# sebhaan/geobo

Hardware: AMD Instinct MI355X
Metric: voxels/sec posterior (mean+var) for 64^3 x 2-prop joint inversion; fp64 roofline % (higher is better)
Workload: dtype f64

## Files before the change

geobo_amd/_lib.py:

```python
import ctypes as C
import os

LIB_PATH = os.environ.get("GEOBO_HIP_LIB") or os.path.join(os.path.dirname(os.path.abspath(__file__)), "lib", "libgeobo_hip.so")

_dp = C.c_void_p
_i64 = C.c_int64
_f64 = C.c_double
_int = C.c_int
_sz = C.c_size_t

SIGNATURES = {
    "geobo_version": (_int, []),
    "geobo_pad_m": (_i64, [_i64]),
    "geobo_pad_n": (_i64, [_i64]),
    "geobo_k_block": (_int, [_int, _dp, _dp, _dp, _i64, _dp, _dp, _dp, _i64, _f64, _f64, _f64, _f64, _dp, _i64, _dp]),
    "geobo_k_block_f32": (_int, [_int, _dp, _dp, _dp, _i64, _dp, _dp, _dp, _i64, _f64, _f64, _f64, _f64, _dp, _i64, _dp]),
    "geobo_k_block_grid": (_int, [_int, _int, _int, _dp, _dp, _i64, _i64, _i64, _i64, _int, _dp, _i64, _dp]),
    "geobo_lattice_wbuild": (_int, [_i64, _int, _int, _int, _dp, _dp, _dp, _dp]),
    "geobo_lattice_wplanes": (_int, [_i64, _int, _int, _int, _dp, _dp, _dp, _dp]),
    "geobo_xz2d_fold_inv_strided": (_int, [_int, _i64, _int, _dp, _i64, _i64, _dp, _dp, _dp, _i64, _i64, _i64, _dp]),
    "geobo_xz2d_fold_inv_mul": (_int, [_int, _i64, _int, _dp, _i64, _dp, _i64, _dp, _dp, _dp, _i64, _i64, _i64, _dp]),
    "geobo_xz2d_fold_conv_fwd": (_int, [_int, _i64, _int, _dp, _i64, _dp, _i64, _dp, _i64, _dp, _dp, _dp, _i64, _i64, _dp]),
    "geobo_sumsq_accum": (_int, [_i64, _i64, _dp, _i64, _dp, _i64, _int, _dp, _i64, _dp]),
    "geobo_lamdot_z": (_int, [_i64, _int, _int, _int, _dp, _dp, _dp, _dp]),
    "geobo_centro_fill": (_int, [_dp, _i64, _i64, _i64, _dp]),
    "geobo_transpose": (_int, [_i64, _i64, _dp, _i64, _dp, _i64, _dp]),
    "geobo_mirror_rows": (_int, [_dp, _i64, _i64, _i64, _i64, _int, _dp]),
    "geobo_mirror_planes": (_int, [_dp, _i64, _dp, _i64, _i64, _i64, _i64, _int, _int, _dp]),
    "geobo_mirror_dev_ws_bytes": (_sz, []),
    "geobo_mirror_dev": (_int, [_dp, _i64, _dp, _i64, _i64, _int, _int, _dp, _dp, _sz, _dp]),
    "geobo_colgemv_ws_bytes": (_sz, [_i64, _i64]),
    "geobo_colgemv": (_int, [_i64, _i64, _dp, _i64, _dp, _dp, _dp, _sz, _dp]),
    "geobo_rowgemv": (_int, [_i64, _i64, _dp, _i64, _dp, _dp, _dp]),
    "geobo_convert": (_int, [_int, _dp, _i64, _dp, _i64, _i64, _i64, _dp]),
    "geobo_round_f32": (_int, [_dp, _i64, _dp]),
    "geobo_k_eval": (_int, [_int, _dp, _i64, _f64, _f64, _f64, _f64, _dp, _dp]),
    "geobo_a_sens": (_int, [_int, C.POINTER(_f64), _dp, _i64, _int, _int, _int, _dp, _dp, _dp, _f64, _f64, _dp, _i64, _dp]),
    "geobo_a_sens_slab": (_int, [_int, C.POINTER(_f64), _dp, _i64, _int, _int, _int, _dp, _dp, _dp, _f64, _f64, _int, _int, _dp, _i64, _i64, _dp]),
    "geobo_potential": (_int, [_int, C.POINTER(_f64), _dp, _dp, _dp, _i64, _dp, _dp]),
    "geobo_ak_fused": (_int, [_int, _dp, _i64, _i64, _i64, _dp, _dp, _dp, _i64, _i64, _f64, _f64, _f64, _f64, _dp, _i64, _dp]),
    "geobo_ak_points": (_int, [_int, _dp, _i64, _i64, _i64, _dp, _dp, _dp, _dp, _dp, _dp, _i64, _f64, _f64, _f64, _f64, _dp, _i64, _dp]),
    "geobo_cov_table": (_int, [_int, _int, _int, _int, _f64, _f64, _f64, _f64, _f64, _f64, _f64, _dp, _dp]),
    "geobo_ak_fused_grid": (_int, [_dp, _i64, _i64, _i64, _int, _int, _int, _dp, _i64, _i64, _dp, _i64, _dp]),
# ... 119 lines not shown
```

geobo_amd/csrc/reduce.hip:

```cpp
#include <hip/hip_runtime.h>
#include <stdint.h>
#include "geobo_hip.h"

namespace {

typedef double v2d __attribute__((ext_vector_type(2)));

__global__ void __launch_bounds__(256) sumsq_accum_kernel(int64_t rows, int64_t n2, const double* __restrict__ a, int64_t lda,
                                                          const double* __restrict__ b, int64_t ldb, int slots, double* __restrict__ ss,
                                                          int64_t ld_ss) {
  const int64_t c2 = (int64_t)blockIdx.x * 256 + threadIdx.x;
  if (c2 >= n2) return;
  const int slot = blockIdx.y;
  v2d acc = *reinterpret_cast<const v2d*>(ss + slot * ld_ss + 2 * c2);
  if (b) {
    for (int64_t r = slot; r < rows; r += slots) {
      const v2d x = *reinterpret_cast<const v2d*>(a + r * lda + 2 * c2) + *reinterpret_cast<const v2d*>(b + r * ldb + 2 * c2);
      acc.x = __builtin_fma(x.x, x.x, acc.x);
      acc.y = __builtin_fma(x.y, x.y, acc.y);
    }
  } else {
    for (int64_t r = slot; r < rows; r += slots) {
      const v2d x = *reinterpret_cast<const v2d*>(a + r * lda + 2 * c2);
      acc.x = __builtin_fma(x.x, x.x, acc.x);
// ... 146 lines not shown

__global__ void __launch_bounds__(256) transpose_kernel(int64_t rows, int64_t cols, const double* __restrict__ src, int64_t lds,
                                                        double* __restrict__ dst, int64_t ldd) {
  __shared__ double t[64][65];
  const int tx = threadIdx.x & 63, ty = threadIdx.x >> 6;
  const int64_t r0 = (int64_t)blockIdx.y * 64, c0 = (int64_t)blockIdx.x * 64;
#pragma unroll 4
  for (int i = ty; i < 64; i += 4)
    if (r0 + i < rows && c0 + tx < cols) t[i][tx] = src[(r0 + i) * lds + c0 + tx];
  __syncthreads();
#pragma unroll 4
  for (int i = ty; i < 64; i += 4)
    if (c0 + i < cols && r0 + tx < rows) dst[(c0 + i) * ldd + r0 + tx] = t[tx][i];
}

}

extern "C" int geobo_transpose(int64_t rows, int64_t cols, const double* src, int64_t lds, double* dst, int64_t ldd, void* stream) {
  if (!src || !dst || rows < 0 || cols < 0 || lds < cols || ldd < rows || (rows + 63) / 64 > 65535) return GEOBO_E_ARG;
  if (rows == 0 || cols == 0) return GEOBO_OK;
  hipLaunchKernelGGL(transpose_kernel, dim3((unsigned)((cols + 63) / 64), (unsigned)((rows + 63) / 64)), dim3(256), 0, (hipStream_t)stream,
                     rows, cols, src, lds, dst, ldd);
  return hipGetLastError() == hipSuccess ? GEOBO_OK : GEOBO_E_LAUNCH;
}

extern "C" int geobo_centro_fill(double* B, int64_t ld, int64_t n, int64_t r0, void* stream) {
  if (!B || ((uintptr_t)B & 15) || n < 0 || r0 < 0 || r0 > n || 2 * r0 < n || ld < n) return GEOBO_E_ARG;
  if (ld & 1) return GEOBO_E_ALIGN;
  if (r0 == n) return GEOBO_OK;
  const int64_t gy = n - r0 < 65535 ? n - r0 : 65535;
// ... 76 lines not shown
```

geobo_amd/csrc/toeplitz.hip:

```cpp
#include <hip/hip_runtime.h>
#include <atomic>
#include <stdint.h>
#include "geobo_hip.h"
#include "lds_optin.h"

namespace {

struct ToeplitzArgs {
  const double* in;
  const double* tab[2];
  double* out[2];
  int64_t C, S, R;
  int nprop, y0, y1;
};

using rsrc_t = __amdgpu_buffer_rsrc_t;
using u32x2 = decltype(__builtin_amdgcn_raw_buffer_load_b64(*static_cast<rsrc_t*>(nullptr), 0, 0, 0));
__device__ __forceinline__ rsrc_t make_rsrc(const double* base, int bytes) {
  return __builtin_amdgcn_make_buffer_rsrc(const_cast<double*>(base), 0, bytes, 0x00020000);
}
__device__ __forceinline__ double ld_lane(rsrc_t rs, unsigned lane8, int soff) {
  return __builtin_bit_cast(double, __builtin_amdgcn_raw_buffer_load_b64(rs, lane8, soff, 0));
}
__device__ __forceinline__ void st_lane(rsrc_t rs, unsigned lane8, int soff, double v) {
// ... 590 lines not shown
  if (C <= 0 || C % 64 || (plane & 1) || (int64_t)ny * plane * 8 >= (1ll << 31)) return GEOBO_E_ALIGN;
  if (ny <= 64) {
    for (int j = 0; j < nprop; j += 2) {
      const int n = nprop - j >= 2 ? 2 : 1;
      const int rc = geobo_toeplitz_y(ny, C, plane, R, n, in, tabs[j], n == 2 ? tabs[j + 1] : nullptr, outs[j], n == 2 ? outs[j + 1] : nullptr,
                                      y0, y1, stream);
      if (rc) return rc;
    }
    return GEOBO_OK;
  }
  ToeplitzWinArgs g;
  g.in = in; g.C = C; g.S = plane; g.R = R; g.nprop = nprop; g.y0 = y0; g.y1 = y1;
  for (int j = 0; j < 3; ++j) { g.tab[j] = tabs[j < nprop ? j : 0]; g.out[j] = outs[j < nprop ? j : 0]; }
  return launch_win_by_ny<false>(ny, g, (hipStream_t)stream);
}
```

geobo_amd/engine.py:

```python
import math
import os
import time

import numpy as np
import torch

from . import geometry, hip
from .plan import COLUMN_FORM_MAX_BYTES, cross_options, cross_rows_route, engine_options, feed_options, gram_gx_route, plan_route
from .columnform import ColumnExchangeMixin
from .rowform import RowFormMixin
from .operators import StreamedOperator
from .transposed import TransposedPosteriorMixin
from .information import SetStatisticsMixin
from .crossval import CrossValidationMixin
from .blocksupport import BlockSupportMixin
from .pointpred import PointPredictionMixin
from .resources import ResourceMixin
from .geobodies import GeobodyMixin
from .intercepts import InterceptMixin
from .append import AppendRowsMixin
from .reweight import ReweightMixin
from .step import Prior, Step
from .sharding import (EmulatedGroup, allreduce_sum_, assemble_columns, backend_of, exchange_blocks, exchange_blocks_finish,
                       exchange_blocks_start, gather_rows, gather_slices, shard_columns)
# ... 119 lines not shown
        self._A = {}
        self._ws = {}
        self._host = {}
        self._auto_denied = set()
        self._pending_exchange = None
        self.use_grid = self.nz >= 16 and self.nz % 2 == 0
        if method not in ("auto", "dense", "spectral"):
            raise ValueError("method must be 'auto', 'dense' or 'spectral'")
        self.method = method
        env = os.environ
        self.route = plan_route(self.nx, self.ny, self.nz, world=world, rank=rank, assembly=assembly, operators=operators, method=method,
                                env=env)
        self.options = engine_options(env)
        self.feed = feed_options(env)
        self.cross = cross_options(env)
        self.use_spectral = self.route.spectral
        if method == "spectral" and not self.use_spectral:
            raise ValueError("spectral method needs grid extents % 16 == 0 and column shards on y-slab boundaries")
        if self.route.operators == "streamed":
            self.streamed = True
        if self.route.note and self.N >= 32768:
            import warnings
            warnings.warn("geobo_amd route %s: %s" % (self.route.describe(), self.route.note), RuntimeWarning, stacklevel=3)
        self._spectral = None
        self._lattice_plan = None
        self._gram, self._lam, self._edgeV = None, {}, {}
        self._lamW, self._edgeVt = {}, {}
        self.aka_mirror_on = self.options.aka_mirror
        self.aka_mirror, self._mirror, self._mirror_meas = {}, {}, None
        self.z_spectrum_on = self.options.z_spectrum
# ... 386 lines not shown
        if self.exchange:
            return self._assemble_AK_spectral_exchange(step, AK)
        kept = ((0, 0), (0, 1), (1, 1))
        run = ((0, 0), (1, 0), (1, 1)) if step.cross_rows == "magn" else kept
        for s_, A in ((0, A_g), (1, A_m)):
            gen_of, out_of = {}, {}
            for jj, j in enumerate(props):
                gen_of[j] = sp.eigenvalues(step.prior.table(self, s_, j))
                step.gens[(s_, j)] = gen_of[j]
                out_of[j] = AK[s_ * self.Ms_pad:s_ * self.Ms_pad + self.Ms, jj * nc:(jj + 1) * nc]
            blocks = [j for j in props if not step.sym or (s_, j) in run]
            lams, outs = [gen_of[j] for j in blocks], [out_of[j] for j in blocks]
            pooled = (isinstance(A, StreamedOperator) and A.lattice is not None and A.lattice.jy is not None and not self.f32
                      and sp.pool_applies())
            Mrun = step.mirror if (s_ == 1 and step.mirror) else self.Ms
            fl = sp.flops(Mrun, len(lams), y1 - y0, fwd_planes=sp.pool_planes(Mrun) if pooled else None)
            fv = sp.flops_valu(Mrun, len(lams), y1 - y0)
            feed = self._gram_feed(step, s_, blocks) if (y0, y1) == (0, self.ny) else None
            if feed is not None:
                fl += self._gram.flops_gx(Mrun * len(lams))

            def product_rows(gx, A=A, lams=lams, outs=outs, Mrun=Mrun, pooled=pooled):
                if not self.f32 and not isinstance(A, StreamedOperator):
                    return sp.product(A, Mrun, lams, [o[:Mrun] for o in outs], y0, y1, gx=gx)
                Rb = sp.R
                abuf = self._op_rows_buffer() if isinstance(A, StreamedOperator) else None
                scr = [self._workspace2d("ak_rows64_%d" % jj, Rb, nc) for jj in range(len(lams))] if self.f32 else None
                pool = sp.plane_pool(A.lattice, Mrun, A.lattice.jy, A.lattice.jx) if pooled else None
                for r0 in range(0, Mrun, Rb):
                    R = min(Rb, Mrun - r0)
                    if pool is not None:
                        src = pool.rows(r0)
                    elif abuf is not None and A.lattice is not None:
                        src = A.lattice.rows(r0)
                    else:
                        src = A.rows_into(abuf, r0, R) if abuf is not None else A[r0:r0 + R]
                    dst = [b[:R] for b in scr] if scr is not None else [o[r0:r0 + R] for o in outs]
                    sp.product(src, R, lams, dst, y0, y1, gx=gx and gx.at(r0))
                    if scr is not None:
                        for jj in range(len(lams)):
                            hip.convert(dst[jj], outs[jj][r0:r0 + R])
            self._timed("spectral_product", fl, lambda: product_rows(feed), valu=fv)
            whole = feed is None or feed.store_all
            late = [j for j in props if (not step.sym or (s_, j) in kept) and not (whole and j in blocks)]
            if late:
                step.ak_fill.append(lambda fill=product_rows, lams=[gen_of[j] for j in late], outs=[out_of[j] for j in late]:
                                    fill(None, lams=lams, outs=outs))

    def _gram_feed(self, step, s_, blocks):
        gram, sp = self._gram, self._spectral_product()
        funcs = ("grav", "magn")
        if not (gram_gx_route(self.feed, self.route.family, step.sym, self.f32, self.world, self.exchange, self.nx, self.ny, self.nz, sp.forms)
                and gram is not None and gram.gx_applies() and sp.gx_applies() and all(j in (0, 1) and self._lam.get(funcs[j]) is not None for j in blocks)):
            return None
        S = [self._workspace("gram_S_%d%d" % (s_, j), (self.Ms * gram.Py * gram.Px,)) for j in blocks]
        for j, Sj in zip(blocks, S):
            step.gram_S[(s_, j)] = Sj
        return _GramFeed(gram, [self._lam[funcs[j]][1] for j in blocks], S, store_all=False)

    def _edge_spectrum(self, func, k, ycols):
        key = (func, k)
        hit = self._edgeV.get(key)
        if hit is None or hit[0] != ycols.data_ptr():
            hit = self._edgeV[key] = (ycols.data_ptr(), self._gram.edge_eigen(ycols))
        return hit[1]

    MIRROR_BOUND = 2.0 ** -48

    def _mirror_static(self, plan):
        return bool(self.aka_mirror_on and plan is not None and plan["rowmajor"] and self.route.family == "single" and self.world == 1
# ... 190 lines not shown
                  props=(0, 1, 2), calclogl=True, want_mean_var=True, keep_K=False, potrf_schedule=None):
        props = tuple(props)
        assert 0 in props and 1 in props, "gravity and magnetic blocks are needed for AkA"
        sel = np.asarray(sel, dtype=np.int64)
        sel_t = torch.as_tensor(sel, device=self.device) if sel.size else None
        t = self._tick("start")
        scales = self._step_row_scale(sel)
        y = self._pad_y(y_g, y_m, y_d, hip.pad_m(2 * self.Ms_pad + len(sel)), None if scales is None else scales[1])
        if self.rows_static and not self._rows_denied and not self._rows_ok(A_g, A_m) and all(f in self._op_args for f in ("grav", "magn")):
            A_g, A_m = (self.operator(f, *self._op_args[f][:1], B=self._op_args[f][1], axes=self._op_args[f][2]) for f in ("grav", "magn"))
        step = self._step = self._new_step(Prior(kernelfunc, lengths, weight_matrix(crossweights), gp_amp), props, sel_t, gp_sigma,
                                           keep_signal=bool(keep_K), row_scale=scales, sym=not self.rows_static and self._sym_ok(A_g, A_m))
        M_pad = step.M_pad
        step.mirror = self._mirror_rows(step, A_m)
        step.cross_rows = "magn" if cross_rows_route(self.cross, step.sym, step.mirror, self.nx, self.ny, self.nz) else "grav"
        for f, rec in self.aka_mirror.items():
            rec["taken"] = bool(f == "magn" and step.mirror)
        AK = self._assemble_AK(step, A_g, A_m)
        self.step_route = "rows" if step.rowpath else ("single" if step.sym else "columns")
        t = self._tick("ak_fused", t)
        AkA = self._assemble_AkA(step, AK, A_g, A_m)
        if self.aka_hook is not None:
            self.aka_hook(AkA)
        t = self._tick("aka", t)
        if self._potrf_ctx is None:
            self._potrf_ctx = hip.PotrfContext()
        Linv, info = self._timed("potrf_inv", 2.0 * M_pad ** 3 / 3.0, lambda: hip.potrf_inv(
            AkA, self._workspace("Linv", (M_pad, M_pad)), self._workspace("potrf_ws", (hip.potrf_ws_doubles(M_pad),)),
            ctx=self._potrf_ctx, schedule=potrf_schedule or self.options.potrf), alg=(2 * self.Ms + len(sel)) ** 3 * 2.0 / 3.0)
        L = AkA
        if scales is not None and scales[1].size:
            Linv.diagonal()[torch.as_tensor(scales[1], device=self.device)] = 0.0
# ... 228 lines not shown
```

geobo_amd/hip.py:

```python
import ctypes as C

import numpy as np
import torch

from . import _lib

F64 = torch.float64

KERNEL_IDS = {"d2": 0, "exp": 1, "exp_x": 2, "matern32": 3, "matern32_x": 4, "sparse": 5, "sparse_x": 6,
              "exp_dl": 7, "exp_x_dl1": 8, "exp_x_dl2": 9, "matern32_dl": 10, "matern32_x_dl1": 11, "matern32_x_dl2": 12,
              "sparse_dl": 13, "sparse_x_dl1": 14, "sparse_x_dl2": 15}
FUNC_IDS = {"grav": 0, "magn": 1}
from .plan import (PAD_M, PAD_N, SPECTRAL_AXIS_N, SPECTRAL_Y3T_NY, SPECTRAL_Y_NY, TOEPLITZ_ADD_NY, TOEPLITZ_NY, TOEPLITZ_Y2T_NY,
                   XZ2D_FOLD_N, XZ2D_SHAPES, YMUL_SHAPES)


def kernel_id(name, cross, deriv=None):
    if name not in ("exp", "matern32", "sparse"):
        raise ValueError("unknown kernelfunc %r (expected 'sparse', 'exp' or 'matern32')" % (name,))
    if deriv is None:
        return KERNEL_IDS[name + ("_x" if cross else "")]
    if isinstance(deriv, bool) or deriv not in (1, 2):
        raise ValueError("deriv must be None, 1 or 2, got %r" % (deriv,))
    if not cross:
# ... 190 lines not shown
def mirror_rows(X, m, r0, nb, nz):
    lib = require_gpu()
    ld = _rowmajor(X, "X")
    assert X.shape[0] >= m and X.shape[1] >= nb * nz
    _lib.check(lib.geobo_mirror_rows(_p(X), int(ld), int(m), int(r0), int(nb), int(nz), _stream()), "geobo_mirror_rows")
    return X


def mirror_planes(src, dst, m, r0, r1, nx, nz):
    lib = require_gpu()
    lds, ldd = _rowmajor(src, "src"), _rowmajor(dst, "dst")
    assert src.shape[0] >= r1 and dst.shape[0] >= m and src.shape[1] >= nx * nz and dst.shape[1] >= nx * nz
    _lib.check(lib.geobo_mirror_planes(_p(src), int(lds), _p(dst), int(ldd), int(m), int(r0), int(r1), int(nx), int(nz), _stream()),
               "geobo_mirror_planes")
    return dst


def mirror_dev_ws_doubles():
    return require_gpu().geobo_mirror_dev_ws_bytes() // 8


def mirror_dev(a, b, rows, nx, nz, out=None, ws=None):
    lib = require_gpu()
    lda, ldb = _rowmajor(a, "a"), _rowmajor(b, "b")
    assert a.shape[0] >= rows and b.shape[0] >= rows
    nws = lib.geobo_mirror_dev_ws_bytes() // 8
    if ws is None:
        ws = torch.empty(nws, dtype=F64, device=a.device)
    if out is None:
        out = torch.empty(2, dtype=F64, device=a.device)
# ... 1081 lines not shown
```

geobo_amd/plan.py:

```python
from dataclasses import asdict, dataclass, make_dataclass

PAD_M, PAD_N = 256, 128
XZ2D_SHAPES = ((48, 64), (64, 64), (64, 32))
XZ2D_FOLD_N = (64,)
TOEPLITZ_NY = (16, 32, 48, 64, 80, 96, 112, 128)
SPECTRAL_AXIS_N = (80, 96, 112, 128)
SPECTRAL_Y_NY = (32, 48, 64, 80, 96, 112, 128)
TOEPLITZ_Y2T_NY = (32, 48, 64)
TOEPLITZ_ADD_NY = (80, 96, 112, 128)
SPECTRAL_Y3T_NY = (80, 96, 112, 128)
YMUL_SHAPES = ((128, 64),)
INTEGER_BASIS_N = (32, 64)
ROWS_MIN_VOXELS = 1 << 18
ROWS_MIN_PLANE = 96 * 96
ROWS_MIN_VOXELS_MID, ROWS_MIN_PLANE_MID = 3 << 17, 64 * 64
COLUMN_FORM_MAX_BYTES = 160 << 30
ROWS_MIN_VOXELS_FUSED = 1 << 17


SWITCHES = {"fused_xz": "GEOBO_SPECTRAL_FUSED_XZ",
            "fold": "GEOBO_XZ_FOLD",
            "quad": "GEOBO_XZ_QUAD",
            "dense_y": "GEOBO_SPECTRAL_DENSE_Y",
            "y_mfma": "GEOBO_Y_MFMA",
# ... 51 lines not shown


CROSS_OPTIONS = {"cross_rows": ("GEOBO_CROSS_ROWS", "auto", _cross_rows)}
CrossOptions = make_dataclass("CrossOptions", [(k, type(d)) for k, (_, d, _p) in CROSS_OPTIONS.items()], frozen=True)


def cross_options(env=None):
    env = {} if env is None else env
    return CrossOptions(**{k: parse(env[var]) if var in env else default for k, (var, default, parse) in CROSS_OPTIONS.items()})


def cross_rows_route(opts, sym, mirror_rows, nx, ny, nz):
    if not (sym and mirror_rows) or opts.cross_rows == "grav":
        return False
    return opts.cross_rows == "magn" or nx == ny == nz == 64


def half_integer(n):
    return n not in INTEGER_BASIS_N


@dataclass(frozen=True)
class Forms:
    xz: str
    x_axis4: bool
    y: str
    y_two_term: str
    y3t: bool
    y2s: bool
    fold: bool
# ... 145 lines not shown
```

geobo_amd/spectral.py:

```python
import math
import os

import numpy as np
import torch

from . import hip, plan
from .plan import INTEGER_BASIS_N, half_integer

F64 = hip.F64
SLACK = 4096


def base_modes(n):
    assert n % 4 == 0
    q = n // 4
    modes = [("cos", 0), ("mid", n // 2), ("cos", q), ("sin", q)]
    for om in range(1, q):
        modes += [("cos", om), ("sin", om), ("cos", n // 2 - om), ("sin", n // 2 - om)]
    return modes


def half_modes(n):
    assert n % 4 == 0
    modes = []
# ... 95 lines not shown
    return jxp * nz + d * ((2 * nx - 1) * nz)


def pool_order(jy, jx):
    return np.lexsort((np.asarray(jy), np.asarray(jx))).astype(np.int32)


def pool_distinct_planes(ny, jy, jx):
    jy, jx = np.asarray(jy, dtype=np.int64), np.asarray(jx, dtype=np.int64)
    d = (ny - 2 - jy)[:, None] + np.arange(1, ny - 1, dtype=np.int64)[None, :]
    return int(np.unique(jx[:, None] * (2 * ny - 3) + d).size) + 2 * int(jy.size)


class PooledRows:

    def __init__(self, pool, row_off, edge, jy, jx, r0=0, geo=None):
        self.pool, self.row_off, self.edge, self.jy, self.jx, self.r0 = pool, row_off, edge, jy, jx, int(r0)
        self.geo = geo if geo is not None else (jy.tobytes(), jx.tobytes())

    def rows(self, r0):
        return PooledRows(self.pool, self.row_off, self.edge, self.jy, self.jx, self.r0 + r0, self.geo)


class ConvolvedRows:

    def __init__(self, gram, Lview, lam3, slab, r0=0):
        self.gram, self.Lview, self.lam3, self.slab, self.r0 = gram, Lview, lam3, slab, int(r0)

    def rows(self, r0):
        return ConvolvedRows(self.gram, self.Lview, self.lam3, self.slab, self.r0 + r0)

    def spectrum(self, sp, R, out_name):
        nx, ny, nz, Px, Py, Cp = sp.nx, sp.ny, sp.nz, sp.Px, sp.Py, sp.Cp
        assert nx == ny == nz == 64 and Cp >= Py * Px
        a = self.r0
        lh = sp.buf("LG_Lh", R * Py * Px)
# ... 54 lines not shown
        n_int, edge_off, edge_row, planes = pool_layout(nx, ny, Ms, Cp)
        buf = self.buf("Pool", planes * Cp)
        hip.xz2d_fold(False, nx, nx, nd, lattice.Q, nz, lattice.q_plane, self.F["x"], self.F["z"], buf, nd * Cp, Cp)
        e0 = lattice.edge[lattice.r0:]
        edge = buf[edge_off:planes * Cp]
        hip.xz2d_fold(False, nx, Ms, 2, e0, lattice.edge.stride(0), nx * nz, self.F["x"], self.F["z"], edge, edge_row, Cp)
        jy, jx = np.ascontiguousarray(jy, dtype=np.int64)[:Ms], np.ascontiguousarray(jx, dtype=np.int64)[:Ms]
        rows = PooledRows(buf, None, edge, jy, jx)
        key = (rows.geo, Cp)
        row_off = self._pool_tabs.get(key)
        if row_off is None:
            row_off = self._pool_tabs[key] = torch.from_numpy(pool_row_off(nx, ny, Cp, jy, jx)).to(self.device)
        rows.row_off = row_off
        return rows

    def _pool_batch(self, A, R):
        a = A.r0
        key = (A.geo, a, R)
        hit = self._pool_tabs.get(key)
        if hit is None:
            jy, jx = A.jy[a:a + R], A.jx[a:a + R]
            hit = self._pool_tabs[key] = (torch.from_numpy(pool_order(jy, jx)).to(self.device), pool_distinct_planes(self.ny, jy, jx))
        return hit

    def _ystage_pooled(self, A, R, tabs, outs, y0, y1):
        ny, C, Cp = self.ny, self.Px * self.Pz, self.Cp
        order, distinct = self._pool_batch(A, R)
        a = A.r0
        fn = lambda: hip.spectral_y_lattice(ny, C, R, A.pool, A.row_off[a:], A.edge[a * 2 * Cp:], 2 * Cp, order, tabs, outs, y0, y1, plane=Cp)
        name = "kernel:toeplitz_y" if len(tabs) >= 2 else "kernel:toeplitz_y_single"
        return self._launch(name, 8.0 * C * (distinct + R * len(tabs) * (y1 - y0)), R, self.y_stage_flop(1, len(tabs), y1 - y0), fn)

    dense_y = property(lambda self: self.forms.y != "spectrum")
    y_mfma = property(lambda self: self.forms.y == "mfma")
    fused_xz = property(lambda self: self.forms.xz in ("fold", "fused"))

    def _ystage(self, R, src, tabs, outs, y0, y1, accumulate=False):
        ny, C, plane = self.ny, self.Px * self.Pz, self.Cp
        if self.y_mfma and (ny > 64 or not accumulate) and (ny <= 64 or 2 * (y1 - y0) >= ny):
            fn = lambda: hip.spectral_y(ny, C, R, src, tabs, outs, y0, y1, plane=plane, accumulate=accumulate)
        else:
            fn = lambda: hip.toeplitz_y(ny, C, R, src, tabs, outs, y0, y1, plane=plane, accumulate=accumulate)
        name = "kernel:toeplitz_y" if len(tabs) >= 2 or ny > 64 else "kernel:toeplitz_y_single"
        return self._launch(name, 8.0 * R * C * (ny + (2 if accumulate else 1) * len(tabs) * (y1 - y0)), R, self.y_stage_flop(1, len(tabs), y1 - y0), fn)
# ... 336 lines not shown
```

geobo_amd/step.py:

```python
from dataclasses import dataclass, field


class Prior:

    def __init__(self, name, lengths, W, amp, deriv=None):
        self.name, self.lengths, self.W, self.amp = name, lengths, W, amp
        self.deriv = None if deriv is None else [float(v) for v in deriv]

    def terms(self, i, j):
        from .hip import kernel_id
        w, d = self.W[i][j], self.deriv
        if d is None:
            return [(kernel_id(self.name, i != j), w)]
        if i == j:
            return [(kernel_id(self.name, False, 1), w * d[j])]
        return [(kernel_id(self.name, True, 1), w * d[j]), (kernel_id(self.name, True, 2), w * d[i])]

    def table(self, eng, i, j):
        tabs = [eng._cov_table(kid, self.lengths[j], self.lengths[i], w, self.amp) for kid, w in self.terms(i, j)]
        for t in tabs[1:]:
            tabs[0].add_(t)
        return tabs[0]

    def k_block(self, eng, i, j, rows, cols, out):
# ... 32 lines not shown
class Step:
    prior: Prior
    props: tuple
    sel_t: object
    Md: int
    M_pad: int
    noise: object = None
    ak_slot: str = "AK"
    aka_slot: str = "AkA"
    keep_signal: bool = False
    row_scale: object = None
    sym: bool = False
    rowpath: bool = False
    mirror: int = 0
    cross_rows: str = "grav"
    gens: dict = field(default_factory=dict)
    fullrows: dict = field(default_factory=dict)
    gram_S: dict = field(default_factory=dict)
    ak_fill: list = field(default_factory=list)
```

geobo_amd/transposed.py:

```python

import torch

from . import hip
from .operators import StreamedOperator

F64 = hip.F64


class TransposedPosteriorMixin:
    def _sym_ok(self, A_g, A_m):
        if not self._zpath_static_ok():
            return False
        return (self._gram is not None and self._gram.edge_supported() and self.Ms_pad == self.nx * self.ny
                and all(self._lam.get(f) is not None and self._lam[f][0] is A for f, A in (("grav", A_g), ("magn", A_m))))

    def _assemble_AkA_sym(self, step, AkA, AK, A_g, A_m):
        gram, pl, ny, Msp, nc = self._gram, self.nx * self.nz, self.ny, self.Ms_pad, self.nc
        Md, off_d, props = step.Md, 2 * self.Ms_pad, step.props
        lam = {0: self._lam["grav"][1], 1: self._lam["magn"][1]}
        ops = {0: A_g, 1: A_m}

        def edge_cols(sp_, k, iy):
            A = ops[sp_]
            if isinstance(A, StreamedOperator):
# ... 15 lines not shown
            slabs(X, nrows, sp_, out)
        blk = lambda r0, j: AK[r0:, props.index(j) * nc:(props.index(j) + 1) * nc]

        Mm = step.mirror or self.Ms
        cross = step.cross_rows == "magn"

        def cross_from_magn():
            X, out, Ms = blk(Msp, 0), AkA[Msp:, 0:Msp], self.Ms
            interior(X, Mm, 0, out, S.get((1, 0)))
            hip.centro_fill(out[:Ms, :Ms], Ms, (Ms + 1) // 2)
            for dst, src in ((0, ny - 1), (ny - 1, 0)):
                hip.mirror_planes(X[:, src * pl:(src + 1) * pl], X[:, dst * pl:(dst + 1) * pl], Ms, 0, Ms - Mm, self.nx, self.nz)
            slabs(X, Ms, 0, out)
            hip.transpose(AkA[Msp:2 * Msp, :Msp], AkA[:Msp, Msp:2 * Msp])

        def run():
            rows_times_AT(blk(0, 0), self.Ms, 0, AkA[0:, 0:Msp], S.get((0, 0)))
            if not cross:
                rows_times_AT(blk(0, 1), self.Ms, 1, AkA[0:, Msp:2 * Msp], S.get((0, 1)))
            rows_times_AT(blk(Msp, 1), Mm, 1, AkA[Msp:, Msp:2 * Msp], S.get((1, 1)))
            if cross:
                cross_from_magn()
            else:
                hip.transpose(AkA[:Msp, Msp:2 * Msp], AkA[Msp:2 * Msp, :Msp])
            if Md:
                rows_times_AT(blk(off_d, 0), Md, 0, AkA[off_d:, 0:Msp])
                rows_times_AT(blk(off_d, 1), Md, 1, AkA[off_d:, Msp:2 * Msp])
        S = step.gram_S
        nfed = sum(self.Ms if s_ == 0 else Mm for s_, _ in S)
        self._timed("aka_lattice", gram.flops((self.Ms + 2 * Mm if cross else 2 * self.Ms + Mm) + 2 * Md - nfed, ny) + gram.flops_back(nfed), run)
        if step.mirror:
            self._timed("aka_centro_fill", 0.0, lambda: hip.centro_fill(AkA[Msp:Msp + self.Ms, Msp:Msp + self.Ms], self.Ms, (self.Ms + 1) // 2))
        return self._finish_AkA(step, AkA)

    def _zpath_static_ok(self):
        if not self.route.single or self.exchange:
            return False
        self._spectral_product()
        return True

    def _zpath_ok(self, step, AK):
        return (self._zpath_static_ok() and AK is not None and AK.dtype == F64
                and all((s_, j) in step.gens for s_ in (0, 1) for j in step.props))

    def _resident_operator(self, A, func):
# ... 207 lines not shown
```

include/geobo_hip.h:

```cpp
#ifndef GEOBO_HIP_H
#define GEOBO_HIP_H

#include <stddef.h>
#include <stdint.h>

#ifdef __cplusplus
extern "C" {
#endif

#define GEOBO_VERSION 213


#define GEOBO_PAD_M 256
#define GEOBO_PAD_N 128

enum { GEOBO_OK = 0, GEOBO_E_ARG = -1, GEOBO_E_ALIGN = -2, GEOBO_E_LAUNCH = -3, GEOBO_E_UNSUPPORTED = -4 };

enum {
  GEOBO_K_D2 = 0,
  GEOBO_K_EXP = 1,
  GEOBO_K_EXP_X = 2,
  GEOBO_K_MATERN32 = 3,
  GEOBO_K_MATERN32_X = 4,
  GEOBO_K_SPARSE = 5,
// ... 187 lines not shown
int geobo_potrf_inv(int64_t m, double* A, int64_t ld, double* Linv, int64_t ldi, int* info, void* ws,
                    size_t ws_bytes, void* ctx, int schedule, void* stream);

int geobo_rowgemv(int64_t m, int64_t n, const double* X, int64_t ld, const double* v, double* out, void* stream);

int geobo_sumsq_accum(int64_t rows, int64_t n, const double* a, int64_t lda, const double* b, int64_t ldb, int slots, double* ss,
                      int64_t ld_ss, void* stream);

int geobo_lamdot_z(int64_t batch, int planes, int px, int nz, const double* D, const double* lam, double* out, void* stream);

int geobo_centro_fill(double* B, int64_t ld, int64_t n, int64_t r0, void* stream);
int geobo_transpose(int64_t rows, int64_t cols, const double* src, int64_t lds, double* dst, int64_t ldd, void* stream);
int geobo_mirror_rows(double* X, int64_t ld, int64_t m, int64_t r0, int64_t nb, int nz, void* stream);
int geobo_mirror_planes(const double* src, int64_t lds, double* dst, int64_t ldd, int64_t m, int64_t r0, int64_t r1, int nx, int nz,
                        void* stream);
size_t geobo_mirror_dev_ws_bytes(void);
int geobo_mirror_dev(const double* a, int64_t lda, const double* b, int64_t ldb, int64_t rows, int nx, int nz, double* out2, void* ws,
                     size_t ws_bytes, void* stream);

size_t geobo_posterior_ws_bytes(int64_t m, int64_t ncols);
int geobo_posterior_reduce(int64_t m, int64_t ncols, const double* Linv, int64_t ldi, const double* AK, int64_t ldak,
                           const double* u, double prior_var, double* mu, double* var, int64_t m_valid, void* ws,
                           size_t ws_bytes, void* stream);

size_t geobo_kinv_dot_ws_bytes(int64_t m, int T);
int geobo_kinv_dot(int64_t m, const double* Linv, int64_t ldl, const double* alpha, int T, const double* const* G, int64_t ldg,
                   const int64_t* seg, double* out, void* ws, size_t ws_bytes, void* stream);

int geobo_trmv_stats(int64_t m, const double* Linv, int64_t ldi, const double* y, const double* L, int64_t ld,
                     double* u, double* stats, void* stream);
// ... 88 lines not shown
```

Before: 2.670 million.

## Exploit centrosymmetry for gravity AkA block using half-row product plus edge corrections

Adds a gravity mirror route. For 64^3 symmetric steps it computes the spectral product for only about half of the gravity rows, with the y-edge planes zeroed. The gravity Gram block is then rebuilt by centro-fill, and the missing edge-plane contributions are restored through new slab_pair_y and sym_add kernels plus mirrored interior planes. The goal is to roughly halve the gravity A*K and A*K*A^T work, at the cost of extra correction passes, added complexity and a risk of numerical or indexing errors.

```diff
diff --git a/geobo_amd/_lib.py b/geobo_amd/_lib.py
--- a/geobo_amd/_lib.py
+++ b/geobo_amd/_lib.py
@@ -27,6 +27,8 @@
     "geobo_transpose": (_int, [_i64, _i64, _dp, _i64, _dp, _i64, _dp]),
     "geobo_mirror_rows": (_int, [_dp, _i64, _i64, _i64, _i64, _int, _dp]),
     "geobo_mirror_planes": (_int, [_dp, _i64, _dp, _i64, _i64, _i64, _i64, _int, _int, _dp]),
+    "geobo_sym_add": (_int, [_i64, _dp, _i64, _dp, _i64, _dp]),
+    "geobo_slab_pair_y": (_int, [_int, _i64, _i64, _i64, _dp, _i64, _dp, _dp, _i64, _dp]),
     "geobo_mirror_dev_ws_bytes": (_sz, []),
     "geobo_mirror_dev": (_int, [_dp, _i64, _dp, _i64, _i64, _int, _int, _dp, _dp, _sz, _dp]),
     "geobo_colgemv_ws_bytes": (_sz, [_i64, _i64]),
diff --git a/geobo_amd/csrc/reduce.hip b/geobo_amd/csrc/reduce.hip
--- a/geobo_amd/csrc/reduce.hip
+++ b/geobo_amd/csrc/reduce.hip
@@ -184,6 +184,27 @@
     if (c0 + i < cols && r0 + tx < rows) dst[(c0 + i) * ldd + r0 + tx] = t[tx][i];
 }
 
+__global__ void __launch_bounds__(256) sym_add_kernel(int64_t n, const double* __restrict__ E, int64_t lde, double* __restrict__ B, int64_t ldb) {
+  __shared__ double t[64][65];
+  const int tx = threadIdx.x & 63, ty = threadIdx.x >> 6;
+  const int64_t r0 = (int64_t)blockIdx.y * 64, c0 = (int64_t)blockIdx.x * 64;
+#pragma unroll 4
+  for (int i = ty; i < 64; i += 4)
+    if (c0 + i < n && r0 + tx < n) t[i][tx] = E[(c0 + i) * lde + r0 + tx];
+  __syncthreads();
+#pragma unroll 4
+  for (int i = ty; i < 64; i += 4)
+    if (r0 + i < n && c0 + tx < n) B[(r0 + i) * ldb + c0 + tx] += E[(r0 + i) * lde + c0 + tx] + t[tx][i];
+}
+
+}
+
+extern "C" int geobo_sym_add(int64_t n, const double* E, int64_t lde, double* B, int64_t ldb, void* stream) {
+  if (!E || !B || n < 0 || lde < n || ldb < n || (n + 63) / 64 > 65535) return GEOBO_E_ARG;
+  if (n == 0) return GEOBO_OK;
+  const unsigned nt = (unsigned)((n + 63) / 64);
+  hipLaunchKernelGGL(sym_add_kernel, dim3(nt, nt), dim3(256), 0, (hipStream_t)stream, n, E, lde, B, ldb);
+  return hipGetLastError() == hipSuccess ? GEOBO_OK : GEOBO_E_LAUNCH;
 }
 
 extern "C" int geobo_transpose(int64_t rows, int64_t cols, const double* src, int64_t lds, double* dst, int64_t ldd, void* stream) {
diff --git a/geobo_amd/csrc/toeplitz.hip b/geobo_amd/csrc/toeplitz.hip
--- a/geobo_amd/csrc/toeplitz.hip
+++ b/geobo_amd/csrc/toeplitz.hip
@@ -628,3 +628,38 @@
   for (int j = 0; j < 3; ++j) { g.tab[j] = tabs[j < nprop ? j : 0]; g.out[j] = outs[j < nprop ? j : 0]; }
   return launch_win_by_ny<false>(ny, g, (hipStream_t)stream);
 }
+
+namespace {
+typedef double sp_v2d __attribute__((ext_vector_type(2)));
+
+__global__ void __launch_bounds__(256) slab_pair_y_kernel(int64_t rows, int64_t C2, int64_t S, const double* __restrict__ in, int64_t in_row,
+                                                          const double* __restrict__ t0, const double* __restrict__ t1, double* __restrict__ out,
+                                                          int64_t out_row) {
+  const int64_t p = (int64_t)blockIdx.x * 256 + threadIdx.x;
+  if (p >= C2) return;
+  const sp_v2d a = reinterpret_cast<const sp_v2d*>(t0)[p], b = reinterpret_cast<const sp_v2d*>(t1)[p];
+#pragma unroll 2
+  for (int64_t r = blockIdx.y; r < rows; r += gridDim.y) {
+    const sp_v2d e0 = reinterpret_cast<const sp_v2d*>(in + r * in_row)[p], e1 = reinterpret_cast<const sp_v2d*>(in + r * in_row + S)[p];
+    sp_v2d o0, o1;
+    o0.x = __builtin_fma(b.x, e1.x, a.x * e0.x);
+    o0.y = __builtin_fma(b.y, e1.y, a.y * e0.y);
+    o1.x = __builtin_fma(a.x, e1.x, b.x * e0.x);
+    o1.y = __builtin_fma(a.y, e1.y, b.y * e0.y);
+    reinterpret_cast<sp_v2d*>(out + r * out_row)[p] = o0;
+    reinterpret_cast<sp_v2d*>(out + r * out_row + S)[p] = o1;
+  }
+}
+}
+
+extern "C" int geobo_slab_pair_y(int ny, int64_t C, int64_t plane, int64_t rows, const double* in, int64_t in_row, const double* tab, double* out,
+                                 int64_t out_row, void* stream) {
+  if (!in || !tab || !out || ny < 2 || rows < 0 || C <= 0 || plane < C || in_row < 2 * plane || out_row < 2 * plane) return GEOBO_E_ARG;
+  if ((C & 1) || (plane & 1) || (in_row & 1) || (out_row & 1) || ((uintptr_t)in & 15) || ((uintptr_t)tab & 15) || ((uintptr_t)out & 15))
+    return GEOBO_E_ALIGN;
+  if (rows == 0) return GEOBO_OK;
+  const int64_t C2 = C / 2, gy = rows < 256 ? rows : 256;
+  hipLaunchKernelGGL(slab_pair_y_kernel, dim3((unsigned)((C2 + 255) / 256), (unsigned)gy), dim3(256), 0, (hipStream_t)stream, rows, C2, plane, in,
+                     in_row, tab, tab + (int64_t)(ny - 1) * C, out, out_row);
+  return hipGetLastError() == hipSuccess ? GEOBO_OK : GEOBO_E_LAUNCH;
+}
diff --git a/geobo_amd/engine.py b/geobo_amd/engine.py
--- a/geobo_amd/engine.py
+++ b/geobo_amd/engine.py
@@ -6,7 +6,8 @@
 import torch
 
 from . import geometry, hip
-from .plan import COLUMN_FORM_MAX_BYTES, cross_options, cross_rows_route, engine_options, feed_options, gram_gx_route, plan_route
+from .plan import (COLUMN_FORM_MAX_BYTES, cross_options, cross_rows_route, engine_options, feed_options, gram_gx_route, grav_mirror_route,
+                   grav_options, plan_route)
 from .columnform import ColumnExchangeMixin
 from .rowform import RowFormMixin
 from .operators import StreamedOperator
@@ -157,6 +158,7 @@
         self.options = engine_options(env)
         self.feed = feed_options(env)
         self.cross = cross_options(env)
+        self.grav = grav_options(env)
         self.use_spectral = self.route.spectral
         if method == "spectral" and not self.use_spectral:
             raise ValueError("spectral method needs grid extents % 16 == 0 and column shards on y-slab boundaries")
@@ -573,19 +575,45 @@
             pooled = (isinstance(A, StreamedOperator) and A.lattice is not None and A.lattice.jy is not None and not self.f32
                       and sp.pool_applies())
             Mrun = step.mirror if (s_ == 1 and step.mirror) else self.Ms
-            fl = sp.flops(Mrun, len(lams), y1 - y0, fwd_planes=sp.pool_planes(Mrun) if pooled else None)
+            half = bool(s_ == 0 and step.grav_mirror)
+            if half:
+                Mrun = step.grav_mirror
+            fl = sp.flops(Mrun, len(lams), y1 - y0, fwd_planes=sp.pool_planes(self.Ms if half else Mrun) if pooled else None)
             fv = sp.flops_valu(Mrun, len(lams), y1 - y0)
             feed = self._gram_feed(step, s_, blocks) if (y0, y1) == (0, self.ny) else None
+            assert not half or ((pooled or not isinstance(A, StreamedOperator)) and feed is not None and not feed.store_all and blocks == [0])
             if feed is not None:
                 fl += self._gram.flops_gx(Mrun * len(lams))
 
-            def product_rows(gx, A=A, lams=lams, outs=outs, Mrun=Mrun, pooled=pooled):
+            def product_rows(gx, A=A, lams=lams, outs=outs, Mrun=Mrun, pooled=pooled, half=half):
+                slabs_to = lambda: self._workspace2d("grav_slabs", self.Ms + 1, 2 * plane)[:self.Ms]
+
+                def keep_planes():
+                    P = self._workspace2d("grav_iplanes", self.Ms + 1, 2 * plane)[:self.Ms]
+                    P[:Mrun, :plane].copy_(outs[0][:Mrun, :plane])
+                    P[:Mrun, plane:].copy_(outs[0][:Mrun, (self.ny - 1) * plane:self.ny * plane])
+                    step.grav_iplanes = P
                 if not self.f32 and not isinstance(A, StreamedOperator):
-                    return sp.product(A, Mrun, lams, [o[:Mrun] for o in outs], y0, y1, gx=gx)
+                    if not half:
+                        return sp.product(A, Mrun, lams, [o[:Mrun] for o in outs], y0, y1, gx=gx)
+                    step.grav_slabs = sp.slab_pair_rows(sp.slab_spectra(A, self.Ms), self.Ms, lams[0], slabs_to())
+                    abuf = self._op_rows_buffer()
+                    for r0 in range(0, Mrun, sp.R):
+                        R = min(sp.R, Mrun - r0)
+                        abuf[:R, :self.N].copy_(A[r0:r0 + R, :self.N])
+                        abuf[:R, :plane].zero_()
+                        abuf[:R, (self.ny - 1) * plane:self.ny * plane].zero_()
+                        sp.product(abuf, R, lams, [o[r0:r0 + R] for o in outs], y0, y1, gx=gx and gx.at(r0))
+                    return keep_planes()
                 Rb = sp.R
                 abuf = self._op_rows_buffer() if isinstance(A, StreamedOperator) else None
                 scr = [self._workspace2d("ak_rows64_%d" % jj, Rb, nc) for jj in range(len(lams))] if self.f32 else None
-                pool = sp.plane_pool(A.lattice, Mrun, A.lattice.jy, A.lattice.jx) if pooled else None
+                pool = sp.plane_pool(A.lattice, self.Ms if half else Mrun, A.lattice.jy, A.lattice.jx) if pooled else None
+                if half:
+                    step.grav_slabs = sp.slab_pair_rows(pool.edge, self.Ms, lams[0], slabs_to())
+                    zero = self._workspace("pool_zero_planes", (2 * sp.Cp,))
+                    zero.zero_()
+                    pool = pool.interior(zero)
                 for r0 in range(0, Mrun, Rb):
                     R = min(Rb, Mrun - r0)
                     if pool is not None:
@@ -599,20 +627,46 @@
                     if scr is not None:
                         for jj in range(len(lams)):
                             hip.convert(dst[jj], outs[jj][r0:r0 + R])
+                if half:
+                    keep_planes()
             self._timed("spectral_product", fl, lambda: product_rows(feed), valu=fv)
             whole = feed is None or feed.store_all
             late = [j for j in props if (not step.sym or (s_, j) in kept) and not (whole and j in blocks)]
             if late:
-                step.ak_fill.append(lambda fill=product_rows, lams=[gen_of[j] for j in late], outs=[out_of[j] for j in late]:
-                                    fill(None, lams=lams, outs=outs))
-
-    def _gram_feed(self, step, s_, blocks):
+                whole_rows = dict(Mrun=self.Ms, half=False) if half else {}
+                step.ak_fill.append(lambda fill=product_rows, lams=[gen_of[j] for j in late], outs=[out_of[j] for j in late], kw=whole_rows:
+                                    fill(None, lams=lams, outs=outs, **kw))
+
+    def _gram_feed_applies(self, step, blocks):
         gram, sp = self._gram, self._spectral_product()
         funcs = ("grav", "magn")
-        if not (gram_gx_route(self.feed, self.route.family, step.sym, self.f32, self.world, self.exchange, self.nx, self.ny, self.nz, sp.forms)
-                and gram is not None and gram.gx_applies() and sp.gx_applies() and all(j in (0, 1) and self._lam.get(funcs[j]) is not None for j in blocks)):
+        return bool(gram_gx_route(self.feed, self.route.family, step.sym, self.f32, self.world, self.exchange, self.nx, self.ny, self.nz, sp.forms)
+                    and gram is not None and gram.gx_applies() and sp.gx_applies()
+                    and all(j in (0, 1) and self._lam.get(funcs[j]) is not None for j in blocks))
+
+    def _grav_mirror_rows(self, step, A_g):
+        if not step.sym:
+            return 0
+        sp = self._spectral_product()
+        hit, lam = self._mirror.get("grav"), self._lam.get("grav")
+        static = hit is not None and hit[0] is A_g
+        even = lam is not None and lam[0] is A_g
+        if isinstance(A_g, StreamedOperator):
+            pooled = A_g.lattice is not None and A_g.lattice.jy is not None and sp.pool_applies()
+        else:
+            pooled = not self.f32
+        pooled = bool(pooled and (self.c0, self.c1) == (0, self.nx * self.ny * self.nz))
+        handover = bool(step.sym and 0 in step.props and self._gram_feed_applies(step, [0]))
+        alone = step.cross_rows == "magn"
+        if not grav_mirror_route(self.grav, step.sym, static, handover, pooled, even, alone, self.nx, self.ny, self.nz):
+            return 0
+        return min(self.Ms, ((self.Ms + 1) // 2 + sp.R - 1) // sp.R * sp.R)
+
+    def _gram_feed(self, step, s_, blocks):
+        gram, funcs = self._gram, ("grav", "magn")
+        if not self._gram_feed_applies(step, blocks):
             return None
-        S = [self._workspace("gram_S_%d%d" % (s_, j), (self.Ms * gram.Py * gram.Px,)) for j in blocks]
+        S =[self._workspace("gram_S_%d%d" % (s_, j), (self.Ms * gram.Py * gram.Px,)) for j in blocks]
         for j, Sj in zip(blocks, S):
             step.gram_S[(s_, j)] = Sj
         return _GramFeed(gram, [self._lam[funcs[j]][1] for j in blocks], S, store_all=False)
@@ -833,8 +887,9 @@
         M_pad = step.M_pad
         step.mirror = self._mirror_rows(step, A_m)
         step.cross_rows = "magn" if cross_rows_route(self.cross, step.sym, step.mirror, self.nx, self.ny, self.nz) else "grav"
+        step.grav_mirror = self._grav_mirror_rows(step, A_g)
         for f, rec in self.aka_mirror.items():
-            rec["taken"] = bool(f == "magn" and step.mirror)
+            rec["taken"] = bool(step.mirror if f == "magn" else step.grav_mirror)
         AK = self._assemble_AK(step, A_g, A_m)
         self.step_route = "rows" if step.rowpath else ("single" if step.sym else "columns")
         t = self._tick("ak_fused", t)
diff --git a/geobo_amd/hip.py b/geobo_amd/hip.py
--- a/geobo_amd/hip.py
+++ b/geobo_amd/hip.py
@@ -228,6 +228,26 @@
     _lib.check(lib.geobo_mirror_planes(_p(src), int(lds), _p(dst), int(ldd), int(m), int(r0), int(r1), int(nx), int(nz), _stream()),
                "geobo_mirror_planes")
     return dst
+
+
+def sym_add(E, B, n):
+    lib = require_gpu()
+    lde, ldb = _rowmajor(E, "E"), _rowmajor(B, "B")
+    assert min(E.shape) >= n and min(B.shape) >= n
+    _lib.check(lib.geobo_sym_add(int(n), _p(E), int(lde), _p(B), int(ldb), _stream()), "geobo_sym_add")
+    return B
+
+
+def slab_pair_y(ny, C, rows, src, tab, out, plane=None):
+    lib = require_gpu()
+    plane = int(C if plane is None else plane)
+    ld = lambda t: t.stride(0) if t.dim() == 2 else 2 * plane
+    room = lambda t: _chk(t, "planes").untyped_storage().nbytes() // 8 - t.storage_offset()
+    assert all(t.dim() == 1 or t.stride(1) == 1 for t in (src, out)) and _chk(tab, "tab").is_contiguous() and tab.numel() >= ny * C
+    assert rows == 0 or min(room(src) - (rows - 1) * ld(src), room(out) - (rows - 1) * ld(out)) >= plane + C
+    _lib.check(lib.geobo_slab_pair_y(int(ny), int(C), plane, int(rows), _p(src), int(ld(src)), _p(tab), _p(out), int(ld(out)), _stream()),
+               "geobo_slab_pair_y")
+    return out
 
 
 def mirror_dev_ws_doubles():
diff --git a/geobo_amd/plan.py b/geobo_amd/plan.py
--- a/geobo_amd/plan.py
+++ b/geobo_amd/plan.py
@@ -89,6 +89,30 @@
     if not (sym and mirror_rows) or opts.cross_rows == "grav":
         return False
     return opts.cross_rows == "magn" or nx == ny == nz == 64
+
+
+GRAV_MIRROR = ("auto", "on", "off")
+
+
+def _grav_mirror(v):
+    if v not in GRAV_MIRROR:
+        raise ValueError("GEOBO_GRAV_MIRROR must be one of %s, got %r" % (", ".join(GRAV_MIRROR), v))
+    return v
+
+
+GRAV_OPTIONS = {"grav_mirror": ("GEOBO_GRAV_MIRROR", "auto", _grav_mirror)}
+GravOptions = make_dataclass("GravOptions", [(k, type(d)) for k, (_, d, _p) in GRAV_OPTIONS.items()], frozen=True)
+
+
+def grav_options(env=None):
+    env = {} if env is None else env
+    return GravOptions(**{k: parse(env[var]) if var in env else default for k, (var, default, parse) in GRAV_OPTIONS.items()})
+
+
+def grav_mirror_route(opts, sym, static, handover, pooled, even, alone, nx, ny, nz):
+    if opts.grav_mirror == "off" or not (sym and static and handover and pooled and even and alone):
+        return False
+    return opts.grav_mirror == "on" or nx == ny == nz == 64
 
 
 def half_integer(n):
diff --git a/geobo_amd/spectral.py b/geobo_amd/spectral.py
--- a/geobo_amd/spectral.py
+++ b/geobo_amd/spectral.py
@@ -133,12 +133,16 @@
 
 class PooledRows:
 
-    def __init__(self, pool, row_off, edge, jy, jx, r0=0, geo=None):
+    def __init__(self, pool, row_off, edge, jy, jx, r0=0, geo=None, edge_row=None):
         self.pool, self.row_off, self.edge, self.jy, self.jx, self.r0 = pool, row_off, edge, jy, jx, int(r0)
         self.geo = geo if geo is not None else (jy.tobytes(), jx.tobytes())
+        self.edge_row = edge_row
 
     def rows(self, r0):
-        return PooledRows(self.pool, self.row_off, self.edge, self.jy, self.jx, self.r0 + r0, self.geo)
+        return PooledRows(self.pool, self.row_off, self.edge, self.jy, self.jx, self.r0 + r0, self.geo, self.edge_row)
+
+    def interior(self, zero_planes):
+        return PooledRows(self.pool, self.row_off, zero_planes, self.jy, self.jx, self.r0, self.geo, 0)
 
 
 class ConvolvedRows:
@@ -223,6 +227,21 @@
         rows.row_off = row_off
         return rows
 
+    def slab_spectra(self, A, Ms):
+        nx, ny, nz, Cp = self.nx, self.ny, self.nz, self.Cp
+        assert self.forms.xz == "fold" and A.stride(1) == 1
+        spec = self.buf("SlabSpec", Ms * 2 * Cp)
+        hip.xz2d_fold(False, nx, Ms, 2, A, A.stride(0), (ny - 1) * nx * nz, self.F["x"], self.F["z"], spec, 2 * Cp, Cp)
+        return spec
+
+    def slab_pair_rows(self, edge_spec, Ms, gen, out):
+        nx, ny, nz, C, Cp = self.nx, self.ny, self.nz, self.Px * self.Pz, self.Cp
+        assert self.forms.xz == "fold" and out.stride(1) == 1 and out.shape[1] >= 2 * nx * nz
+        spec = self.buf("S", Ms * 2 * Cp)
+        hip.slab_pair_y(ny, C, Ms, edge_spec, gen, spec, plane=Cp)
+        hip.xz2d_fold(True, nx, Ms, 2, spec, 2 * Cp, Cp, self.F["x"], self.F["z"], out, out.stride(0), nx * nz)
+        return out
+
     def _pool_batch(self, A, R):
         a = A.r0
         key = (A.geo, a, R)
@@ -236,7 +255,8 @@
         ny, C, Cp = self.ny, self.Px * self.Pz, self.Cp
         order, distinct = self._pool_batch(A, R)
         a = A.r0
-        fn = lambda: hip.spectral_y_lattice(ny, C, R, A.pool, A.row_off[a:], A.edge[a * 2 * Cp:], 2 * Cp, order, tabs, outs, y0, y1, plane=Cp)
+        er = 2 * Cp if A.edge_row is None else A.edge_row
+        fn = lambda: hip.spectral_y_lattice(ny, C, R, A.pool, A.row_off[a:], A.edge[a * er:], er, order, tabs, outs, y0, y1, plane=Cp)
         name = "kernel:toeplitz_y" if len(tabs) >= 2 else "kernel:toeplitz_y_single"
         return self._launch(name, 8.0 * C * (distinct + R * len(tabs) * (y1 - y0)), R, self.y_stage_flop(1, len(tabs), y1 - y0), fn)
 
diff --git a/geobo_amd/step.py b/geobo_amd/step.py
--- a/geobo_amd/step.py
+++ b/geobo_amd/step.py
@@ -70,7 +70,10 @@
     rowpath: bool = False
     mirror: int = 0
     cross_rows: str = "grav"
+    grav_mirror: int = 0
     gens: dict = field(default_factory=dict)
     fullrows: dict = field(default_factory=dict)
     gram_S: dict = field(default_factory=dict)
+    grav_slabs: object = None
+    grav_iplanes: object = None
     ak_fill: list = field(default_factory=list)
diff --git a/geobo_amd/transposed.py b/geobo_amd/transposed.py
--- a/geobo_amd/transposed.py
+++ b/geobo_amd/transposed.py
@@ -53,8 +53,27 @@
             slabs(X, Ms, 0, out)
             hip.transpose(AkA[Msp:2 * Msp, :Msp], AkA[:Msp, Msp:2 * Msp])
 
+        Mg = step.grav_mirror or self.Ms
+
+        def grav_from_half():
+            P, out, Ms = step.grav_iplanes, AkA[0:, 0:Msp], self.Ms
+            gram.back_rows(S[(0, 0)], Mg, out)
+            hip.centro_fill(out[:Ms, :Ms], Ms, (Ms + 1) // 2)
+            for dst, src in ((0, 1), (1, 0)):
+                hip.mirror_planes(P[:, src * pl:(src + 1) * pl], P[:, dst * pl:(dst + 1) * pl], Ms, 0, Ms - Mg, self.nx, self.nz)
+            E = self._workspace2d("grav_E", Ms, Ms)
+            E.zero_()
+            for k, iy in enumerate((0, ny - 1)):
+                gram.edge_rows(P[:, k * pl:], Ms, self._edge_spectrum("grav", k, edge_cols(0, k, iy)), E)
+            hip.sym_add(E, out[:Ms, :Ms], Ms)
+            for k, iy in enumerate((0, ny - 1)):
+                gram.edge_rows(step.grav_slabs[:, k * pl:], Ms, self._edge_spectrum("grav", k, edge_cols(0, k, iy)), out)
+
         def run():
-            rows_times_AT(blk(0, 0), self.Ms, 0, AkA[0:, 0:Msp], S.get((0, 0)))
+            if step.grav_mirror:
+                grav_from_half()
+            else:
+                rows_times_AT(blk(0, 0), self.Ms, 0, AkA[0:, 0:Msp], S.get((0, 0)))
             if not cross:
                 rows_times_AT(blk(0, 1), self.Ms, 1, AkA[0:, Msp:2 * Msp], S.get((0, 1)))
             rows_times_AT(blk(Msp, 1), Mm, 1, AkA[Msp:, Msp:2 * Msp], S.get((1, 1)))
@@ -66,8 +85,8 @@
                 rows_times_AT(blk(off_d, 0), Md, 0, AkA[off_d:, 0:Msp])
                 rows_times_AT(blk(off_d, 1), Md, 1, AkA[off_d:, Msp:2 * Msp])
         S = step.gram_S
-        nfed = sum(self.Ms if s_ == 0 else Mm for s_, _ in S)
-        self._timed("aka_lattice", gram.flops((self.Ms + 2 * Mm if cross else 2 * self.Ms + Mm) + 2 * Md - nfed, ny) + gram.flops_back(nfed), run)
+        nfed = sum(Mg if s_ == 0 else Mm for s_, _ in S)
+        self._timed("aka_lattice", gram.flops((Mg + 2 * Mm if cross else 2 * self.Ms + Mm) + 2 * Md - nfed, ny) + gram.flops_back(nfed), run)
         if step.mirror:
             self._timed("aka_centro_fill", 0.0, lambda: hip.centro_fill(AkA[Msp:Msp + self.Ms, Msp:Msp + self.Ms], self.Ms, (self.Ms + 1) // 2))
         return self._finish_AkA(step, AkA)
diff --git a/include/geobo_hip.h b/include/geobo_hip.h
--- a/include/geobo_hip.h
+++ b/include/geobo_hip.h
@@ -225,6 +225,9 @@
 int geobo_mirror_rows(double* X, int64_t ld, int64_t m, int64_t r0, int64_t nb, int nz, void* stream);
 int geobo_mirror_planes(const double* src, int64_t lds, double* dst, int64_t ldd, int64_t m, int64_t r0, int64_t r1, int nx, int nz,
                         void* stream);
+int geobo_sym_add(int64_t n, const double* E, int64_t lde, double* B, int64_t ldb, void* stream);
+int geobo_slab_pair_y(int ny, int64_t C, int64_t plane, int64_t rows, const double* in, int64_t in_row, const double* tab, double* out,
+                      int64_t out_row, void* stream);
 size_t geobo_mirror_dev_ws_bytes(void);
 int geobo_mirror_dev(const double* a, int64_t lda, const double* b, int64_t ldb, int64_t rows, int nx, int nz, double* out2, void* ws,
                      size_t ws_bytes, void* stream);
```

After: 2.837 million (median of 6 runs). +6.3%, better.
